# jizongFox/MI-based-Regularized-Semi-supervised-Segmentation

Measured on AMD Instinct MI355X. Metric: images/sec (UNet+IIC fwd/bwd) ACDC 256^2, higher is better.
Workload: dtype bf16; 1 GPU; udaiic train step, ACDC-shaped 1x256x256 4-class slices, LB=UB=16 per GPU, taps Conv5/Up_conv3/Up_conv2, K=20 x 5 sub-heads, paddings [1,3] (BASELINE configs[1]); mi_precision=f16f8, global_batch=32, parallelism=dp1, launch_tape=True, tape_ops=170, tape_replays_in_run=449

## Files before the change

mi-based-regularized-semi-supervised-segmentation_amd/csrc/api.hip:

```cpp
#include <stdarg.h>

#include "common.h"

namespace miseg_core {
static thread_local char g_err[512] = "";
char* last_error_buf() { return g_err; }
int fail(int code, const char* fmt, ...) {
    va_list ap;
    va_start(ap, fmt);
    vsnprintf(g_err, sizeof(g_err), fmt, ap);
    va_end(ap);
    return code;
}
}

extern "C" int miseg_version(void) { return 406; }
extern "C" const char* miseg_last_error(void) { return miseg::last_error_buf(); }

namespace miseg_core {
static hipEvent_t next_fork_event() {
    constexpr int kRing = 256, kDev = 16;
    struct Ring { hipEvent_t ev[kRing]; int made = 0, next = 0; };
    static thread_local Ring rings[kDev];
    int dev = 0;
    if (hipGetDevice(&dev) != hipSuccess || dev < 0 || dev >= kDev) return nullptr;
    Ring& r = rings[dev];
    constexpr unsigned flags = hipEventDisableTiming | hipEventDisableSystemFence;
    if (r.made < kRing) {
        if (hipEventCreateWithFlags(&r.ev[r.made], flags) != hipSuccess) return nullptr;
        ++r.made;
    }
    hipEvent_t ev = r.ev[r.next % r.made];
    r.next = (r.next + 1) % kRing;
    return ev;
}
}

extern "C" int miseg_stream_wait_stream(void* waiter, void* producer) {
    MISEG_TAPE(miseg_stream_wait_stream, waiter, producer);
    if (waiter == producer) return MISEG_OK;
    hipEvent_t ev = miseg_core::next_fork_event();
    if (!ev) return miseg_core::fail(MISEG_E_LAUNCH, "stream_wait_stream: hipEventCreateWithFlags failed");
    hipError_t e = hipEventRecord(ev, reinterpret_cast<hipStream_t>(producer));
    if (e == hipSuccess) e = hipStreamWaitEvent(reinterpret_cast<hipStream_t>(waiter), ev, 0);
    if (e != hipSuccess) return miseg_core::fail(MISEG_E_LAUNCH, "stream_wait_stream: %s", hipGetErrorString(e));
    return MISEG_OK;
}
```

mi-based-regularized-semi-supervised-segmentation_amd/csrc/conv.hip:

```cpp
#include "common.h"

namespace miseg {

constexpr int kCT = 256;
constexpr int TH = 16;
constexpr int CK = 32;

template <typename T> struct Mma;
template <> struct Mma<bf16> {
    static constexpr int CKP = 40;
    static constexpr int KP = 48;
    static constexpr int VEC = 8;
    typedef s16x8 Frag;
    static __device__ __forceinline__ Frag load(const bf16* base, int kq) { return *reinterpret_cast<const Frag*>(base + 8 * kq); }
    static __device__ __forceinline__ void mma_chunk(const Frag& a, const Frag& b, f32x4& c) {
        c = __builtin_amdgcn_mfma_f32_16x16x32_bf16(a, b, c, 0, 0, 0);
    }
};
template <> struct Mma<float> {
    static constexpr int CKP = 34;
    static constexpr int KP = 34;
    static constexpr int VEC = 4;
    struct Frag { float v[8]; };
    static __device__ __forceinline__ Frag load(const float* base, int kq) {
        Frag f;
#pragma unroll
        for (int s = 0; s < 8; ++s) f.v[s] = base[4 * s + kq];
        return f;
    }
    static __device__ __forceinline__ void mma_chunk(const Frag& a, const Frag& b, f32x4& c) {
#pragma unroll
        for (int s = 0; s < 8; ++s) c = __builtin_amdgcn_mfma_f32_16x16x4f32(a.v[s], b.v[s], c, 0, 0, 0);
    }
};

struct ConvSrc {
    const void* p0; const void* p1;
    int C0, C1, ups0, ups1;
};

template <typename T>
__device__ __forceinline__ void zero_vec(T* dst) {
#pragma unroll
    for (int i = 0; i < Mma<T>::VEC; ++i) dst[i] = from_f32<T>(0.f);
}

template <typename T, int COT, int TW, int THT, bool POOL = false, bool BNL = false, bool RED = false, int NW = 4>
__global__ __launch_bounds__(64 * NW, 1) void conv3x3_kernel(ConvSrc src, int N, int H, int W, const T* __restrict__ wpk, int Cout,
                                                        T* __restrict__ out, float* __restrict__ stats, BnFinish fin, BnLoad bl, BnRed br) {
    static_assert(!(RED && POOL), "the epilogue reduce exists for full-resolution outputs");
    typedef Mma<T> MM;
    constexpr int kCT = 64 * NW;
    static_assert(THT % NW == 0, "whole rows per wave");
    constexpr int VEC = MM::VEC, NT = COT / 16, MTR = TW / 16, RW = THT / NW, MTW = RW * MTR;
    constexpr int KP = MM::KP;
    constexpr int IW = TW + 2, IH = THT + 2;
    constexpr int NIS = (IH * IW * (CK / VEC) + kCT - 1) / kCT, NWS = (9 * COT * (CK / VEC) + kCT - 1) / kCT;
    extern __shared__ __attribute__((aligned(16))) unsigned char smem[];
    T* Is = reinterpret_cast<T*>(smem);
    T* Ws = Is + IH * IW * KP;
    const int Cin = src.C0 + src.C1;
    const int tid = threadIdx.x, lane = tid & 63, wv = tid >> 6, l15 = lane & 15, kq = lane >> 4;
    const int tilesC = (W + TW - 1) / TW, tilesR = (H + THT - 1) / THT;
    const int tc = blockIdx.x % tilesC, tr = (blockIdx.x / tilesC) % tilesR, n = blockIdx.x / (tilesC * tilesR);
    const int h0 = tr * THT, w0 = tc * TW, co0 = blockIdx.y * COT;

    f32x4 acc[MTW][NT];
#pragma unroll
    for (int m = 0; m < MTW; ++m)
#pragma unroll
        for (int t = 0; t < NT; ++t) acc[m][t] = f32x4{0.f, 0.f, 0.f, 0.f};

    uint4 pin[NIS], pwt[NWS];
    uint4 pgy[BNL ? NIS : 1];
    float cfr[BNL ? kBwdCoefRows * VEC : 1];
    unsigned okm = 0;
    static_assert(NIS <= 32 && kCT % (CK / VEC) == 0, "slot mask / per-thread channel vector");
    const uint4 zero4 = make_uint4(0u, 0u, 0u, 0u);
    auto fetch = [&](int c0) __attribute__((always_inline)) {
        if (BNL) {
            okm = 0;
            const int c = c0 + (tid % (CK / VEC)) * VEC;
#pragma unroll
// ... 370 lines not shown
                            float v = acc[m0][t][r] + acc[m1][t][r];
                            v += __shfl_xor(v, 1, 64);
                            pk[r] = from_f32<T>(v);
                        }
                        if (!mine) continue;
                        if (co + 3 < Cout) *reinterpret_cast<uint2*>(op + co) = *reinterpret_cast<const uint2*>(pk);
                        else {
#pragma unroll
                            for (int r = 0; r < 4; ++r)
                                if (co + r < Cout) op[co + r] = pk[r];
                        }
                    }
                }
            } else {
#pragma unroll
                for (int m = 0; m < MTW; ++m) {
                    const int h = h0 + wv * RW + m / MTR, w = w0 + (m % MTR) * 16 + l15;
                    const bool ok = h < H && w < W;
                    const size_t px = ((size_t)n * H + h) * W + w;
#pragma unroll
                    for (int t = 0; t < NT; ++t) {
                        const int co = co0 + t * 16 + kq * 4;
                        T* op = out + px * Cout;
                        if (fin.out1) op = co < fin.split ? out + px * fin.split : reinterpret_cast<T*>(fin.out1) + px * (Cout - fin.split) - fin.split;
                        if (ok && co + 3 < Cout) {
                            T pk[4];
#pragma unroll
                            for (int r = 0; r < 4; ++r) {
                                const float v = acc[m][t][r];
                                pk[r] = from_f32<T>(v);
                                s1[t][r] += v;
                                s2[t][r] += v * v;
                            }
                            *reinterpret_cast<uint2*>(op + co) = *reinterpret_cast<const uint2*>(pk);
                        } else if (ok) {
#pragma unroll
                            for (int r = 0; r < 4; ++r)
                                if (co + r < Cout) {
                                    const float v = acc[m][t][r];
                                    op[co + r] = from_f32<T>(v);
                                    s1[t][r] += v;
                                    s2[t][r] += v * v;
                                }
                        }
                    }
                }
            }
        }
        advance(p);
    };
    while (p.tile < t_end) {
        stage(pinA, pwtA);
        if constexpr (DEPTH == 2) {
            if (p.tile >= t_end) break;
            stage(pinB, pwtB);
        }
    }
    if (!POOL && stats) {
        __shared__ float sred[NW][2][COT];
#pragma unroll
        for (int t = 0; t < NT; ++t)
#pragma unroll
            for (int r = 0; r < 4; ++r) {
                float a = s1[t][r], b = s2[t][r];
#pragma unroll
                for (int off = 1; off < 16; off <<= 1) {
                    a += __shfl_xor(a, off, 64);
                    b += __shfl_xor(b, off, 64);
                }
                if (l15 == 0) { sred[wv][0][t * 16 + kq * 4 + r] = a; sred[wv][1][t * 16 + kq * 4 + r] = b; }
            }
        __syncthreads();
        if (tid < COT && co0 + tid < Cout) {
            float a = sred[0][0][tid] + sred[1][0][tid] + sred[2][0][tid] + sred[3][0][tid];
            float b = sred[0][1][tid] + sred[1][1][tid] + sred[2][1][tid] + sred[3][1][tid];
#pragma unroll
            for (int q = 4; q < NW; ++q) { a += sred[q][0][tid]; b += sred[q][1][tid]; }
            if (fin.acc) {
                bn_acc_add(fin.acc + co0 + tid, fin.acc + 2 * Cout, a);
                bn_acc_add(fin.acc + Cout + co0 + tid, fin.acc + 2 * Cout, b);
            } else {
                stats[((size_t)blockIdx.x * 2 + 0) * Cout + co0 + tid] = a;
                stats[((size_t)blockIdx.x * 2 + 1) * Cout + co0 + tid] = b;
            }
        }
    }
}

typedef unsigned int u32x4v __attribute__((ext_vector_type(4)));
template <int COT, int TW, int NVEC, bool DUAL, bool POOL = false, bool BNL = false, bool RED = false, int RW = 4>
__global__ __launch_bounds__(kCT, 2) void conv3x3_stream_kernel(ConvSrc src, int N, int H, int W, const bf16* __restrict__ wpk, int Cout,
                                                               bf16* __restrict__ out, float* __restrict__ stats, int ntiles, BnFinish fin,
                                                               BnLoad bl, BnRed br) {
    typedef bf16 T;
    typedef Mma<T> MM;
    static_assert(!BNL || (!DUAL && (NVEC == 1 || NVEC == 2 || NVEC == 4)), "BN loader: one source, a thread keeps one channel vector");
    static_assert(!(RED && POOL), "the epilogue reduce exists for full-resolution outputs");
    constexpr int THS = 4 * RW;
    static_assert(RW == 2 || RW == 4, "rows per wave");
    constexpr int CKP = MM::CKP, VEC = MM::VEC, NT = COT / 16, MTR = TW / 16, MTW = RW * MTR;
    constexpr int IKP = COT == 16 ? 48 : CKP;
    constexpr int IW = TW + 2, IH = THS + 2, NPIX = IH * IW;
    constexpr int NPF = DUAL ? NVEC * ((NPIX + kCT - 1) / kCT) : (NPIX * NVEC + kCT - 1) / kCT;
    constexpr unsigned OOB = 0xFFFFFF00u;
    extern __shared__ __attribute__((aligned(16))) unsigned char smem[];
    T* Is = reinterpret_cast<T*>(smem);
    T* Ws = Is + IH * IW * IKP;
    float* Cf = reinterpret_cast<float*>(Ws + 9 * COT * CKP);
    float* Rf = Cf + (BNL ? kBwdCoefRows * CK : 0);
    const int Cin = src.C0 + src.C1;
    const int tid = threadIdx.x, lane = tid & 63, wv = tid >> 6, l15 = lane & 15, kq = lane >> 4;
    const int tilesC = (W + TW - 1) / TW, tilesR = (H + THS - 1) / THS;
    const int co0 = blockIdx.y * COT;
    const int G = gridDim.x;
    const int lb = (G % 8 == 0) ? (int)(blockIdx.x % 8) * (G / 8) + (int)(blockIdx.x / 8) : (int)blockIdx.x;
    if (BNL)
        for (int idx = tid; idx < kBwdCoefRows * CK; idx += kCT) {
            const int r = idx / CK, c = idx % CK;
            Cf[idx] = c < Cin ? bl.coef[(size_t)r * Cin + c] : 0.f;
        }
    if (RED)
        for (int idx = tid; idx < 3 * COT; idx += kCT) {
            const int r = idx / COT, c = co0 + idx % COT;
            Rf[idx] = c < Cout ? br.saved[(size_t)(r == 0 ? 0 : r + 1) * Cout + c] : 0.f;
        }

    for (int idx = tid; idx < NPIX * (CK / VEC); idx += kCT) {
        const int v = idx % (CK / VEC), px = idx / (CK / VEC);
        if (v >= NVEC) zero_vec<T>(Is + px * IKP + v * VEC);
    }
    for (int idx = tid; idx < 9 * COT * (CK / VEC); idx += kCT) {
        const int v = idx % (CK / VEC), co = (idx / (CK / VEC)) % COT, tap = idx / ((CK / VEC) * COT);
        const int c = v * VEC;
        T* dst = Ws + (tap * COT + co) * CKP + v * VEC;
        if (co0 + co >= Cout || c >= Cin) { zero_vec<T>(dst); continue; }
        *reinterpret_cast<uint4*>(dst) = *reinterpret_cast<const uint4*>(wpk + ((size_t)tap * Cout + co0 + co) * Cin + c);
    }

    const int hs0 = H >> src.ups0, ws0 = W >> src.ups0, hs1 = H >> src.ups1, ws1 = W >> src.ups1;
    unsigned rel[NPF], yx[NPF];
#pragma unroll
    for (int j = 0; j < NPF; ++j) {
        int v, px;
        if (DUAL) { v = j % NVEC; px = tid + kCT * (j / NVEC); }
        else { const int idx = tid + kCT * j; v = idx % NVEC; px = idx / NVEC; }
        const int ix = px % IW, iy = px / IW, c = v * VEC;
        const bool used = px < NPIX;
        const bool from1 = c >= src.C0;
        const int ups = from1 ? src.ups1 : src.ups0, wsz = from1 ? ws1 : ws0, Cs = from1 ? src.C1 : src.C0, cs = from1 ? c - src.C0 : c;
        const int ry = ((iy - 1) >> ups) + 1, rx = ((ix - 1) >> ups) + 1;
        rel[j] = (unsigned)(((ry * wsz + rx) * Cs + cs) * 2);
        yx[j] = (used ? (unsigned)(iy | (ix << 8)) : 0xFFFFu) | ((unsigned)(used ? px * IKP + v * VEC : 0) << 16);
        static_assert(NPIX * IKP < 65536, "ldso must fit 16 bits");
    }

    if (BNL || RED) __syncthreads();
    u32x4v pf[NPF];
    u32x4v pg[BNL ? NPF : 1];
    auto fetch = [&](int tile) __attribute__((always_inline)) {
        const int tc = tile % tilesC, tr = (tile / tilesC) % tilesR, n = tile / (tilesC * tilesR);
        const int h0 = tr * THS, w0 = tc * TW;
        const int ylo = h0 == 0 ? 1 : 0, yhi = min(IH, H - h0 + 1), xlo = w0 == 0 ? 1 : 0, xhi = min(IW, W - w0 + 1);
        const long long b0 = ((((long long)n * hs0 + (h0 >> src.ups0) - 1) * ws0 + (w0 >> src.ups0) - 1) * src.C0) * 2;
        const __amdgpu_buffer_rsrc_t r0 = __builtin_amdgcn_make_buffer_rsrc((void*)((const char*)src.p0 + b0), 0, 0x7FFFFFFF, 0x00020000);
        __amdgpu_buffer_rsrc_t r1 = r0;
        if (DUAL) {
// ... 955 lines not shown
        for (int m = 0; m < ppb; ++m) t += swr[(m * G + gg) * 37 + tap * 4 + r];
        partials[(size_t)blockIdx.x * Cout * 9 + o] = t;
    }
}
__global__ __launch_bounds__(256) void stem_wgrad_sum_kernel(const float* __restrict__ partials, int nparts, int len, float* __restrict__ gw) {
    reduce_partials_block(partials, nparts, (size_t)len, len, gw, [](int e) { return (size_t)e; });
}
constexpr int kStemBlocksMax = 4096;
static const int kStemBlocks = [] { const char* e = getenv("MISEG_STEM_BLOCKS"); return e ? std::min(kStemBlocksMax, std::max(1, atoi(e))) : 1024; }();

static inline int tile_w(int64_t W) { return W >= 32 ? 32 : 16; }

}

using namespace miseg;

extern "C" int miseg_pack_conv3x3_weights(void* stream, int dt, const float* w, int64_t Cout, int64_t Cin, int kind, int64_t ci_begin,
                                          int64_t ci_count, void* packed) {
    MISEG_TAPE(miseg_pack_conv3x3_weights, stream, dt, w, Cout, Cin, kind, ci_begin, ci_count, packed);
    MISEG_F16_DISPATCH_ON(dt, miseg_pack_conv3x3_weights, stream, MISEG_BF16, w, Cout, Cin, kind, ci_begin, ci_count, packed);
    MISEG_REQUIRE(w && packed && Cout > 0 && Cin > 0, "pack_conv3x3_weights: bad args");
    MISEG_REQUIRE(kind >= 0 && (kind & 0xff) <= 1 && (kind >> 8) <= Cin && (!(kind >> 8) || !(kind & 0xff)), "pack_conv3x3_weights: bad kind");
    if (!(kind & 0xff)) { ci_begin = 0; ci_count = Cin; }
    MISEG_REQUIRE(ci_begin >= 0 && ci_count > 0 && ci_begin + ci_count <= Cin, "pack_conv3x3_weights: bad channel slice");
    const int total = (int)(9 * ((kind & 0xff) ? ci_count * Cout : Cout * Cin));
    const int nb = std::min((total + 255) / 256, 1024);
    if (dt == MISEG_F32)
        hipLaunchKernelGGL(pack_w_kernel<float>, dim3(nb), dim3(256), 0, as_stream(stream), w, (int)Cout, (int)Cin, kind, (int)ci_begin, (int)ci_count, (float*)packed);
    else if (dt == MISEG_BF16)
        hipLaunchKernelGGL(pack_w_kernel<bf16>, dim3(nb), dim3(256), 0, as_stream(stream), w, (int)Cout, (int)Cin, kind, (int)ci_begin, (int)ci_count, (bf16*)packed);
    else return fail(MISEG_E_INVALID, "pack_conv3x3_weights: bad dtype");
    MISEG_LAUNCH_CHECK("pack_w_kernel");
    return MISEG_OK;
}

extern "C" int miseg_pack_conv3x3_weights_multi(void* stream, int dt, const void* jobs_dev, int64_t njobs, int64_t total_blocks) {
    MISEG_TAPE(miseg_pack_conv3x3_weights_multi, stream, dt, jobs_dev, njobs, total_blocks);
    MISEG_F16_DISPATCH_ON(dt, miseg_pack_conv3x3_weights_multi, stream, MISEG_BF16, jobs_dev, njobs, total_blocks);
    MISEG_REQUIRE(jobs_dev && njobs > 0 && total_blocks > 0, "pack_conv3x3_weights_multi: bad args");
    static_assert(sizeof(PackJob) == 40, "PackJob layout must match miseg_pack_job");
    if (dt == MISEG_F32)
        hipLaunchKernelGGL(pack_w_multi_kernel<float>, dim3((unsigned)total_blocks), dim3(256), 0, as_stream(stream), (const PackJob*)jobs_dev, (int)njobs);
    else if (dt == MISEG_BF16)
        hipLaunchKernelGGL(pack_w_multi_kernel<bf16>, dim3((unsigned)total_blocks), dim3(256), 0, as_stream(stream), (const PackJob*)jobs_dev, (int)njobs);
    else return fail(MISEG_E_INVALID, "pack_conv3x3_weights_multi: bad dtype");
    MISEG_LAUNCH_CHECK("pack_w_multi_kernel");
    return MISEG_OK;
}

namespace miseg {
__global__ __launch_bounds__(256) void slice_cin_kernel(const float* __restrict__ src, int Cout, int Cin_pad, int Cin, float* __restrict__ dst) {
    const int total = Cout * Cin * 9;
    for (int e = blockIdx.x * 256 + threadIdx.x; e < total; e += gridDim.x * 256) {
        const int t = e % 9, ci = (e / 9) % Cin, co = e / (9 * Cin);
        dst[e] = src[((size_t)co * Cin_pad + ci) * 9 + t];
    }
}
}
extern "C" int miseg_conv3x3_wgrad_slice(void* stream, const float* gw_padded, int64_t Cout, int64_t Cin_pad, int64_t Cin, float* gw) {
    MISEG_TAPE(miseg_conv3x3_wgrad_slice, stream, gw_padded, Cout, Cin_pad, Cin, gw);
    MISEG_REQUIRE(gw_padded && gw && Cout > 0 && Cin > 0 && Cin <= Cin_pad, "conv3x3_wgrad_slice: bad args");
    const int total = (int)(Cout * Cin * 9);
    hipLaunchKernelGGL(slice_cin_kernel, dim3(std::min((total + 255) / 256, 256)), dim3(256), 0, as_stream(stream), gw_padded, (int)Cout, (int)Cin_pad,
                       (int)Cin, gw);
    MISEG_LAUNCH_CHECK("slice_cin_kernel");
    return MISEG_OK;
}

static bool conv_streams(int dt, int64_t Cin, int64_t N, int64_t H, int64_t W) {
    return dt == MISEG_BF16 && Cin <= CK && tile_w(W) == 32 && N * cdiv(H, TH) * cdiv(W, 32) >= 512;
}
static int64_t stream_blocks(int64_t N, int64_t H, int64_t W) {
    static const int64_t cap = [] { const char* e = getenv("MISEG_STREAM_BLOCKS"); return e ? atoll(e) : 512LL; }();
    return std::min<int64_t>(N * cdiv(H, TH) * cdiv(W, 32), cap);
}

struct PtGrid { int blocks, per; };
static inline PtGrid pt_grid(int ntiles, int slices, int th) {
    static const int per_cu = [] { const char* e = getenv("MISEG_PT_BLOCKS_PER_CU"); return e ? std::max(1, atoi(e)) : 2; }();
    const int target = std::max(1, (256 * (th == 8 ? per_cu : 1)) / std::max(1, slices));
    const int per = std::max(1, (ntiles + target - 1) / target);
    return PtGrid{(ntiles + per - 1) / per, per};
}
static inline bool tiled_persistent() {
    static const bool on = [] { const char* e = getenv("MISEG_CONV_PERSISTENT"); return !e || atoi(e) != 0; }();
    return on;
}

static int generic_tile_h(int dt, int64_t H, int64_t W) {
    if (dt != MISEG_BF16) return 16;
    return H * W >= 64 * 64 ? 8 : 16;
}

extern "C" int64_t miseg_conv3x3_stats_parts(int dt, int64_t Cin, int64_t N, int64_t H, int64_t W) {
    MISEG_F16_DISPATCH_ON(dt, miseg_conv3x3_stats_parts, MISEG_BF16, Cin, N, H, W);
    if (conv_streams(dt, Cin, N, H, W)) return stream_blocks(N, H, W);
    const int tw = tile_w(W);
    return N * cdiv(H, generic_tile_h(dt, H, W)) * cdiv(W, tw);
}

extern "C" int64_t miseg_conv3x3_fwd_parts(int dt, int64_t Cin, int64_t N, int64_t H, int64_t W, int64_t Cout) {
    MISEG_F16_DISPATCH_ON(dt, miseg_conv3x3_fwd_parts, MISEG_BF16, Cin, N, H, W, Cout);
    const int64_t ntiles = miseg_conv3x3_stats_parts(dt, Cin, N, H, W);
    if (conv_streams(dt, Cin, N, H, W) || dt != MISEG_BF16 || !tiled_persistent()) return ntiles;
    const int th = generic_tile_h(dt, H, W);
    if (th != 8) return ntiles;
    const int64_t cot = Cout <= 16 ? 16 : 32;
    return pt_grid((int)ntiles, (int)cdiv(Cout, cot), th).blocks;
}

static bool sumpool_supported(int dt, int64_t Cin, int64_t N, int64_t H, int64_t W, int64_t Cout) {
    if (H % 2 || W % 2) return false;
    return conv_streams(dt, Cin, N, H, W) || (dt == MISEG_BF16 && Cout > 32);
}

template <typename TT, int COT, int TWW, int THH, bool POOL>
static void launch_tiled(dim3 grid, hipStream_t st, const ConvSrc& s, int N, int H, int W, const void* wpk, int Cout, void* out, float* stats,
                         const BnFinish& fin, const BnLoad& bl, const BnRed& br) {
    const size_t lb = ((size_t)(THH + 2) * (TWW + 2) + 9 * COT) * Mma<TT>::KP * sizeof(TT);
    if constexpr (sizeof(TT) == 2) {
        if (THH == 8 && !bl.gy && !br.raw && !fin.counter && tiled_persistent()) {
            const int ntiles = (int)grid.x;
            const PtGrid g = pt_grid(ntiles, (int)grid.y, THH);
            constexpr int NWW = (THH == 16) ? 8 : 4;
            static const int depth = [] { const char* e = getenv("MISEG_CONV_DEPTH"); return e ? atoi(e) : 1; }();
            if (depth == 2 && !POOL) {
                hipFuncSetAttribute((const void*)conv3x3_pt_kernel<TT, COT, TWW, THH, POOL, NWW, 2>, hipFuncAttributeMaxDynamicSharedMemorySize, (int)lb);
                hipLaunchKernelGGL((conv3x3_pt_kernel<TT, COT, TWW, THH, POOL, NWW, 2>), dim3((unsigned)g.blocks, grid.y), dim3(64 * NWW), lb, st, s, N, H, W,
                                   (const TT*)wpk, Cout, (TT*)out, stats, fin, ntiles, g.per);
            } else {
                hipFuncSetAttribute((const void*)conv3x3_pt_kernel<TT, COT, TWW, THH, POOL, NWW, 1>, hipFuncAttributeMaxDynamicSharedMemorySize, (int)lb);
                hipLaunchKernelGGL((conv3x3_pt_kernel<TT, COT, TWW, THH, POOL, NWW, 1>), dim3((unsigned)g.blocks, grid.y), dim3(64 * NWW), lb, st, s, N, H, W,
                                   (const TT*)wpk, Cout, (TT*)out, stats, fin, ntiles, g.per);
            }
            return;
        }
    }
#define GO(BNL, RED, NWW)                                                                                                            \
    {                                                                                                                               \
        hipFuncSetAttribute((const void*)conv3x3_kernel<TT, COT, TWW, THH, POOL, BNL, RED, NWW>, hipFuncAttributeMaxDynamicSharedMemorySize, (int)lb); \
        hipLaunchKernelGGL((conv3x3_kernel<TT, COT, TWW, THH, POOL, BNL, RED, NWW>), grid, dim3(64 * NWW), lb, st, s, N, H, W, (const TT*)wpk, \
                           Cout, (TT*)out, stats, fin, bl, br);                                                                     \
    }
    if constexpr (THH == 16 && sizeof(TT) == 2) {
        if (!bl.gy && !br.raw) { GO(false, false, 8) return; }
    }
    if constexpr (POOL) { if (bl.gy) GO(true, false, 4) else GO(false, false, 4) }
    else { if (bl.gy && br.raw) GO(true, true, 4) else if (bl.gy) GO(true, false, 4) else if (br.raw) GO(false, true, 4) else GO(false, false, 4) }
#undef GO
}
template <int COT, int NV, bool POOL> constexpr int fused_rw() { return (NV == 2 && (COT == 16 || POOL)) ? 4 : 2; }
template <int COT, int NV, bool DU, bool POOL>
static int launch_stream(unsigned blocks, hipStream_t st, const ConvSrc& s, int N, int H, int W, const void* wpk, int Cout, void* out, float* stats,
                         const BnFinish& fin, const BnLoad& bl, const BnRed& br) {
    const dim3 grid(blocks, (unsigned)cdiv(Cout, COT));
#define GO(BNL, RED, RWW)                                                                                                            \
    {                                                                                                                               \
        const size_t lb = ((size_t)(4 * RWW + 2) * (32 + 2) * (COT == 16 ? 48 : Mma<bf16>::CKP) + 9 * COT * Mma<bf16>::CKP) * sizeof(bf16) + \
                          (BNL ? kBwdCoefRows * CK * 4 : 0) + (RED ? 3 * COT * 4 : 0);                                               \
        const int ntiles = (int)(N * cdiv(H, 4 * RWW) * cdiv(W, 32));                                                                \
        hipFuncSetAttribute((const void*)conv3x3_stream_kernel<COT, 32, NV, DU, POOL, BNL, RED, RWW>, hipFuncAttributeMaxDynamicSharedMemorySize, (int)lb); \
        hipLaunchKernelGGL((conv3x3_stream_kernel<COT, 32, NV, DU, POOL, BNL, RED, RWW>), grid, dim3(kCT), lb, st, s, N, H, W,          \
                           (const bf16*)wpk, Cout, (bf16*)out, stats, ntiles, fin, bl, br);                                          \
    }
    constexpr bool kFusable = !DU && (NV == 2 || NV == 4);
    if constexpr (kFusable) {
        constexpr int FRW = fused_rw<COT, NV, POOL>();
        if constexpr (POOL) { if (bl.gy) GO(true, false, FRW) else GO(false, false, 4) }
        else { if (bl.gy && br.raw) GO(true, true, FRW) else if (bl.gy) GO(true, false, FRW) else if (br.raw) GO(false, true, FRW) else GO(false, false, 4) }
    } else {
        if (bl.gy || br.raw) return fail(MISEG_E_INVALID, "conv3x3: BatchNorm loader / reduce not built for this streaming shape");
        GO(false, false, 4)
    }
#undef GO
    return MISEG_OK;
}

static int conv3x3_fwd_impl(void* stream, int dt, const void* in0, int64_t C0, int ups0, const void* in1, int64_t C1, int ups1,
                            int64_t N, int64_t H, int64_t W, const void* packed_w, int64_t Cout, void* out, float* stats, BnFinish fin,
                            bool pool_out = false, BnLoad bl = BnLoad{nullptr, nullptr}, BnRed br = BnRed{nullptr, nullptr, nullptr}) {
    MISEG_REQUIRE(in0 && packed_w && out, "conv3x3_fwd: null pointer");
    MISEG_REQUIRE(N > 0 && H > 0 && W > 0 && Cout > 0 && C0 > 0 && C1 >= 0, "conv3x3_fwd: bad shape");
    MISEG_REQUIRE(C1 == 0 || in1, "conv3x3_fwd: second source missing");
    MISEG_REQUIRE((ups0 == 0 || ups0 == 1) && (ups1 == 0 || ups1 == 1), "conv3x3_fwd: ups must be 0/1");
    MISEG_REQUIRE((!ups0 || (H % 2 == 0 && W % 2 == 0)) && (!ups1 || (H % 2 == 0 && W % 2 == 0)), "conv3x3_fwd: upsampled size must be even");
    const int vec = dt == MISEG_BF16 ? 8 : 4;
    MISEG_REQUIRE(C0 % vec == 0 && C1 % vec == 0, "conv3x3_fwd: channel counts must be multiples of %d (use conv_small for the stem)", vec);
    ConvSrc s{in0, in1, (int)C0, (int)C1, ups0, ups1};
    const int tw = tile_w(W);
    const int th = conv_streams(dt, C0 + C1, N, H, W) ? TH : generic_tile_h(dt, H, W);
    const unsigned gx = (unsigned)(N * cdiv(H, th) * cdiv(W, tw));
    hipStream_t st = as_stream(stream);
    MISEG_REQUIRE(!bl.gy || (bl.coef && C1 == 0 && ups0 == 0), "conv3x3: the BatchNorm loader reads one full-resolution source");
    MISEG_REQUIRE(!br.raw || (br.saved && br.parts && !pool_out && !stats && Cout % 4 == 0), "conv3x3: epilogue reduce needs a full-resolution "
                  "output with a multiple of 4 channels and no forward statistics");
#define LAUNCH_TH(TT, COT, TWW, THH)                                                                                       \
    launch_tiled<TT, COT, TWW, THH, false>(dim3(gx, (unsigned)cdiv(Cout, COT)), st, s, (int)N, (int)H, (int)W, packed_w, (int)Cout, out, stats, fin, bl, br);
#define LAUNCH(TT, COT, TWW) { if (th == 8) LAUNCH_TH(TT, COT, TWW, 8) else LAUNCH_TH(TT, COT, TWW, 16) }
    MISEG_REQUIRE(!pool_out || (sumpool_supported(dt, C0 + C1, N, H, W, Cout) && C1 == 0 && !stats),
                  "conv3x3_fwd_sumpool: shape not supported (ask miseg_conv3x3_fwd_sumpool_supported)");
    if (conv_streams(dt, C0 + C1, N, H, W)) {
        int rc = MISEG_OK;
#define SLAUNCH(COT, NV, DU)                                                                                               \
    {                                                                                                                     \
        const unsigned g = (unsigned)stream_blocks(N, H, W);                                                               \
        if (pool_out && !DU) rc = launch_stream<COT, NV, false, true>(g, st, s, (int)N, (int)H, (int)W, packed_w, (int)Cout, out, stats, fin, bl, br); \
        else rc = launch_stream<COT, NV, DU, false>(g, st, s, (int)N, (int)H, (int)W, packed_w, (int)Cout, out, stats, fin, bl, br); \
    }
#define SLAUNCH_NV(COT)                                                                                                    \
    {                                                                                                                     \
        if (C1 > 0) { switch ((C0 + C1) / 8) { case 2: SLAUNCH(COT, 2, true) break; case 3: SLAUNCH(COT, 3, true) break; default: SLAUNCH(COT, 4, true) break; } } \
        else { switch (C0 / 8) { case 1: SLAUNCH(COT, 1, false) break; case 2: SLAUNCH(COT, 2, false) break; case 3: SLAUNCH(COT, 3, false) break; default: SLAUNCH(COT, 4, false) break; } } \
    }
        if (Cout <= 16) SLAUNCH_NV(16)
        else SLAUNCH_NV(32)
#undef SLAUNCH_NV
#undef SLAUNCH
        if (rc != MISEG_OK) return rc;
    } else if (dt == MISEG_BF16 && pool_out) {
#define LAUNCH_P(TWW, THH)                                                                                                 \
    launch_tiled<bf16, 64, TWW, THH, true>(dim3(gx, (unsigned)cdiv(Cout, 64)), st, s, (int)N, (int)H, (int)W, packed_w, (int)Cout, out, stats, fin, bl, br);
        if (tw == 32) { if (th == 8) LAUNCH_P(32, 8) else LAUNCH_P(32, 16) }
        else { if (th == 8) LAUNCH_P(16, 8) else LAUNCH_P(16, 16) }
#undef LAUNCH_P
    } else if (dt == MISEG_BF16) {
// ... 293 lines not shown
```

Before: 4947 images/s.

## Add double-buffered tiled 3x3 conv kernel overlapping global loads with MFMA

Adds a new tiled conv3x3 kernel that keeps two shared-memory buffers, one per input-channel chunk. Global loads for chunk k+2 are issued into registers and committed to the spare buffer tap by tap while MFMAs run on the current chunk, so there is one barrier per chunk. It is enabled by default (through an env toggle) for 16-row, 16-bit tiled convs that have no BN loader, no reduce and no counter. The cost is roughly double the LDS footprint at one block per CU and extra register pressure from the staged loads. A standalone per-layer benchmark script is also added.

```diff
diff --git a/mi-based-regularized-semi-supervised-segmentation_amd/csrc/api.hip b/mi-based-regularized-semi-supervised-segmentation_amd/csrc/api.hip
--- a/mi-based-regularized-semi-supervised-segmentation_amd/csrc/api.hip
+++ b/mi-based-regularized-semi-supervised-segmentation_amd/csrc/api.hip
@@ -14,7 +14,7 @@
 }
 }
 
-extern "C" int miseg_version(void) { return 406; }
+extern "C" int miseg_version(void) { return 407; }
 extern "C" const char* miseg_last_error(void) { return miseg::last_error_buf(); }
 
 namespace miseg_core {
diff --git a/mi-based-regularized-semi-supervised-segmentation_amd/csrc/conv.hip b/mi-based-regularized-semi-supervised-segmentation_amd/csrc/conv.hip
--- a/mi-based-regularized-semi-supervised-segmentation_amd/csrc/conv.hip
+++ b/mi-based-regularized-semi-supervised-segmentation_amd/csrc/conv.hip
@@ -1,4 +1,5 @@
 #include "common.h"
+#include <type_traits>
 
 namespace miseg {
 
@@ -535,6 +536,238 @@
             } else {
                 stats[((size_t)blockIdx.x * 2 + 0) * Cout + co0 + tid] = a;
                 stats[((size_t)blockIdx.x * 2 + 1) * Cout + co0 + tid] = b;
+            }
+        }
+    }
+}
+
+template <typename T, int COT, int TW, int THT, bool POOL, int NW>
+__global__ __launch_bounds__(64 * NW, 1) void conv3x3_db_kernel(ConvSrc src, int N, int H, int W, const T* __restrict__ wpk, int Cout,
+                                                           T* __restrict__ out, float* __restrict__ stats, BnFinish fin) {
+    static_assert(sizeof(T) == 2, "double-buffered tiled form: 16-bit storage types");
+    typedef Mma<T> MM;
+    constexpr int kCT = 64 * NW;
+    static_assert(THT % NW == 0, "whole rows per wave");
+    constexpr int VEC = MM::VEC, CV4 = CK / VEC, NT = COT / 16, MTR = TW / 16, RW = THT / NW, MTW = RW * MTR;
+    constexpr int KS = CK;
+    constexpr int IW = TW + 2, IH = THT + 2;
+    constexpr int NIS = (IH * IW * CV4 + kCT - 1) / kCT, NWS = (9 * COT * CV4 + kCT - 1) / kCT, NSL = NIS + NWS;
+    constexpr int RPS = kCT / CV4;
+    static_assert(RPS % 8 == 0 && RPS % COT == 0 && NIS <= 16 && NWS <= 16, "slot j of a thread: same swizzle term, same output channel as slot 0");
+    constexpr int IMG = (IH * IW + 9 * COT) * KS;
+    static_assert((IH * IW) % 4 == 0 && NSL <= 18, "the weight block starts on a 256-byte bank row; two slots per tap");
+    extern __shared__ __attribute__((aligned(16))) unsigned char smem[];
+    T* S = reinterpret_cast<T*>(smem);
+    const int Cin = src.C0 + src.C1;
+    const int tid = threadIdx.x, lane = tid & 63, wv = tid >> 6, l15 = lane & 15, kq = lane >> 4;
+    const int tilesC = (W + TW - 1) / TW, tilesR = (H + THT - 1) / THT;
+    const int tc = blockIdx.x % tilesC, tr = (blockIdx.x / tilesC) % tilesR, n = blockIdx.x / (tilesC * tilesR);
+    const int h0 = tr * THT, w0 = tc * TW, co0 = blockIdx.y * COT;
+    const int nck = (Cin + CK - 1) / CK;
+
+    const int cv = (tid % CV4) * VEC, row0 = tid / CV4;
+    const int sofs = row0 * KS + (cv ^ ((((row0 >> 2) & 1) << 1) * VEC));
+    int i_rel0[NIS], i_rel1[NIS];
+    unsigned okm = 0, wkm = 0;
+    {
+        const int ws0 = W >> src.ups0, ws1 = W >> src.ups1;
+#pragma unroll
+        for (int j = 0; j < NIS; ++j) {
+            const int px = row0 + RPS * j, h = h0 - 1 + px / IW, w = w0 - 1 + px % IW;
+            if (px < IH * IW && h >= 0 && h < H && w >= 0 && w < W) okm |= 1u << j;
+            i_rel0[j] = ((h >> src.ups0) * ws0 + (w >> src.ups0)) * src.C0 + cv;
+            i_rel1[j] = ((h >> src.ups1) * ws1 + (w >> src.ups1)) * src.C1 + cv - src.C0;
+        }
+#pragma unroll
+        for (int j = 0; j < NWS; ++j)
+            if (row0 + RPS * j < 9 * COT && co0 + row0 % COT < Cout) wkm |= 1u << j;
+    }
+    const T* s0n = reinterpret_cast<const T*>(src.p0) + (size_t)n * (H >> src.ups0) * (W >> src.ups0) * src.C0;
+    const T* s1n = reinterpret_cast<const T*>(src.p1) + (size_t)n * (H >> src.ups1) * (W >> src.ups1) * src.C1;
+    const T* wrow = wpk + ((size_t)(row0 / COT) * Cout + co0 + row0 % COT) * Cin + cv;
+    const size_t wstep = (size_t)(RPS / COT) * Cout * Cin;
+
+    uint4 pin[NIS], pwt[NWS];
+    auto slot_ok = [&](int s, int c0) __attribute__((always_inline)) {
+        return (s < NIS ? (okm >> s) & 1u : (wkm >> (s - NIS)) & 1u) && c0 + cv < Cin;
+    };
+    auto fetch_slot = [&](int s, int c0) __attribute__((always_inline)) {
+        const bool ok = slot_ok(s, c0);
+        if (s < NIS) {
+            const bool first = c0 + cv < src.C0;
+            const T* a = ok ? (first ? s0n + i_rel0[s] : s1n + i_rel1[s]) + c0 : s0n;
+            pin[s] = *reinterpret_cast<const uint4*>(a);
+        } else {
+            const int j = s - NIS;
+            const T* a = ok ? wrow + j * wstep + c0 : wpk;
+            pwt[j] = *reinterpret_cast<const uint4*>(a);
+        }
+    };
+    auto keep = [](bool ok, const uint4& q) __attribute__((always_inline)) {
+        return make_uint4(ok ? q.x : 0u, ok ? q.y : 0u, ok ? q.z : 0u, ok ? q.w : 0u);
+    };
+    auto commit_slot = [&](int s, int c0, T* img) __attribute__((always_inline)) {
+        const bool ok = slot_ok(s, c0);
+        if (s < NIS) {
+            if (row0 + RPS * s < IH * IW) *reinterpret_cast<uint4*>(img + sofs + s * RPS * KS) = keep(ok, pin[s]);
+        } else {
+            const int j = s - NIS;
+            if (row0 + RPS * j < 9 * COT) *reinterpret_cast<uint4*>(img + IH * IW * KS + sofs + j * RPS * KS) = keep(ok, pwt[j]);
+        }
+    };
+    int ibase[8];
+    {
+        const int R0 = wv * RW * IW + l15;
+#pragma unroll
+        for (int c7 = 0; c7 < 8; ++c7) {
+            const int r = R0 + c7;
+            ibase[c7] = r * KS + ((kq ^ (((r >> 2) & 1) << 1)) * VEC);
+        }
+    }
+    const int wbase = IH * IW * KS + l15 * KS + ((kq ^ (((l15 >> 2) & 1) << 1)) * VEC);
+
+    f32x4 acc[MTW][NT];
+#pragma unroll
+    for (int m = 0; m < MTW; ++m)
+#pragma unroll
+        for (int t = 0; t < NT; ++t) acc[m][t] = f32x4{0.f, 0.f, 0.f, 0.f};
+
+#pragma unroll
+    for (int s = 0; s < NSL; ++s) fetch_slot(s, 0);
+#pragma unroll
+    for (int s = 0; s < NSL; ++s) commit_slot(s, 0, S);
+    if (nck > 1) {
+#pragma unroll
+        for (int s = 0; s < NSL; ++s) fetch_slot(s, CK);
+    }
+    __syncthreads();
+    auto body = [&](int k, auto wr_c, auto ld_c) __attribute__((always_inline)) {
+        constexpr bool WR = decltype(wr_c)::value, LD = decltype(ld_c)::value;
+        const T* cur = S + (k & 1) * IMG;
+        T* nxt = S + ((k + 1) & 1) * IMG;
+#pragma unroll
+        for (int tap = 0; tap < 9; ++tap) {
+            if constexpr (WR) {
+#pragma unroll
+                for (int s = 0; s < NSL; ++s)
+                    if (8 - (NSL - 1 - s) / 2 == tap) {
+                        commit_slot(s, (k + 1) * CK, nxt);
+                        if constexpr (LD) fetch_slot(s, (k + 2) * CK);
+                    }
+            }
+            const int ky = tap / 3, kx = tap % 3;
+            typename MM::Frag bf[NT];
+#pragma unroll
+            for (int t = 0; t < NT; ++t) bf[t] = *reinterpret_cast<const typename MM::Frag*>(cur + wbase + (tap * COT + t * 16) * KS);
+#pragma unroll
+            for (int m = 0; m < MTW; ++m) {
+                const int c = (m / MTR + ky) * IW + (m % MTR) * 16 + kx;
+                typename MM::Frag af = *reinterpret_cast<const typename MM::Frag*>(cur + ibase[c & 7] + (c & ~7) * KS);
+#pragma unroll
+                for (int t = 0; t < NT; ++t) MM::mma_chunk(bf[t], af, acc[m][t]);
+            }
+        }
+        __syncthreads();
+    };
+    {
+        int k = 0;
+        for (; k + 2 < nck; ++k) body(k, std::true_type{}, std::true_type{});
+        if (k + 1 < nck) body(k++, std::true_type{}, std::false_type{});
+        body(k, std::false_type{}, std::false_type{});
+    }
+    if (POOL) {
+        static_assert(!POOL || RW % 2 == 0, "pooled epilogue: a wave owns whole row pairs");
+        const int Hp = H >> 1, Wp = W >> 1;
+#pragma unroll
+        for (int mp = 0; mp < MTW / 2; ++mp) {
+            const int m0 = (2 * (mp / MTR)) * MTR + mp % MTR, m1 = m0 + MTR;
+            const int hp = ((h0 + wv * RW) >> 1) + mp / MTR, wp = ((w0 + (mp % MTR) * 16) >> 1) + (l15 >> 1);
+            const bool mine = !(l15 & 1) && hp < Hp && wp < Wp;
+            T* op = out + (((size_t)n * Hp + hp) * Wp + wp) * Cout;
+#pragma unroll
+            for (int t = 0; t < NT; ++t) {
+                const int co = co0 + t * 16 + kq * 4;
+                T pk[4];
+#pragma unroll
+                for (int r = 0; r < 4; ++r) {
+                    float v = acc[m0][t][r] + acc[m1][t][r];
+                    v += __shfl_xor(v, 1, 64);
+                    pk[r] = from_f32<T>(v);
+                }
+                if (!mine) continue;
+                if (co + 3 < Cout) *reinterpret_cast<uint2*>(op + co) = *reinterpret_cast<const uint2*>(pk);
+                else {
+#pragma unroll
+                    for (int r = 0; r < 4; ++r)
+                        if (co + r < Cout) op[co + r] = pk[r];
+                }
+            }
+        }
+        return;
+    }
+    float s1[NT][4], s2[NT][4];
+#pragma unroll
+    for (int t = 0; t < NT; ++t)
+#pragma unroll
+        for (int r = 0; r < 4; ++r) s1[t][r] = s2[t][r] = 0.f;
+#pragma unroll
+    for (int m = 0; m < MTW; ++m) {
+        const int h = h0 + wv * RW + m / MTR, w = w0 + (m % MTR) * 16 + l15;
+        const bool ok = h < H && w < W;
+        const size_t px = ((size_t)n * H + h) * W + w;
+#pragma unroll
+        for (int t = 0; t < NT; ++t) {
+            const int co = co0 + t * 16 + kq * 4;
+            T* op = out + px * Cout;
+            if (fin.out1) op = co < fin.split ? out + px * fin.split : reinterpret_cast<T*>(fin.out1) + px * (Cout - fin.split) - fin.split;
+            if (ok && co + 3 < Cout) {
+                T pk[4];
+#pragma unroll
+                for (int r = 0; r < 4; ++r) {
+                    const float v = acc[m][t][r];
+                    pk[r] = from_f32<T>(v);
+                    s1[t][r] += v;
+                    s2[t][r] += v * v;
+                }
+                *reinterpret_cast<uint2*>(op + co) = *reinterpret_cast<const uint2*>(pk);
+            } else if (ok) {
+#pragma unroll
+                for (int r = 0; r < 4; ++r)
+                    if (co + r < Cout) {
+                        const float v = acc[m][t][r];
+                        op[co + r] = from_f32<T>(v);
+                        s1[t][r] += v;
+                        s2[t][r] += v * v;
+                    }
+            }
+        }
+    }
+    if (stats) {
+        __shared__ float sred[NW][2][COT];
+#pragma unroll
+        for (int t = 0; t < NT; ++t)
+#pragma unroll
+            for (int r = 0; r < 4; ++r) {
+                float a = s1[t][r], b = s2[t][r];
+#pragma unroll
+                for (int off = 1; off < 16; off <<= 1) {
+                    a += __shfl_xor(a, off, 64);
+                    b += __shfl_xor(b, off, 64);
+                }
+                if (l15 == 0) { sred[wv][0][t * 16 + kq * 4 + r] = a; sred[wv][1][t * 16 + kq * 4 + r] = b; }
+            }
+        __syncthreads();
+        if (tid < COT && co0 + tid < Cout) {
+            float a = sred[0][0][tid] + sred[1][0][tid] + sred[2][0][tid] + sred[3][0][tid];
+            float b = sred[0][1][tid] + sred[1][1][tid] + sred[2][1][tid] + sred[3][1][tid];
+#pragma unroll
+            for (int q = 4; q < NW; ++q) { a += sred[q][0][tid]; b += sred[q][1][tid]; }
+            if (fin.acc) {
+                bn_acc_add(fin.acc + co0 + tid, fin.acc + 2 * Cout, a);
+                bn_acc_add(fin.acc + Cout + co0 + tid, fin.acc + 2 * Cout, b);
+            } else {
+                store_part(&stats[((size_t)blockIdx.x * 2 + 0) * Cout + co0 + tid], a);
+                store_part(&stats[((size_t)blockIdx.x * 2 + 1) * Cout + co0 + tid], b);
             }
         }
     }
@@ -1656,6 +1889,10 @@
     const int per = std::max(1, (ntiles + target - 1) / target);
     return PtGrid{(ntiles + per - 1) / per, per};
 }
+static inline bool tiled_pipeline() {
+    const char* e = getenv("MISEG_CONV_PIPELINE");
+    return !e || atoi(e) != 0;
+}
 static inline bool tiled_persistent() {
     static const bool on = [] { const char* e = getenv("MISEG_CONV_PERSISTENT"); return !e || atoi(e) != 0; }();
     return on;
@@ -1715,6 +1952,15 @@
         hipFuncSetAttribute((const void*)conv3x3_kernel<TT, COT, TWW, THH, POOL, BNL, RED, NWW>, hipFuncAttributeMaxDynamicSharedMemorySize, (int)lb); \
         hipLaunchKernelGGL((conv3x3_kernel<TT, COT, TWW, THH, POOL, BNL, RED, NWW>), grid, dim3(64 * NWW), lb, st, s, N, H, W, (const TT*)wpk, \
                            Cout, (TT*)out, stats, fin, bl, br);                                                                     \
+    }
+    if constexpr (THH == 16 && sizeof(TT) == 2) {
+        if (!bl.gy && !br.raw && !fin.counter && tiled_pipeline()) {
+            const size_t lb2 = 2 * ((size_t)(THH + 2) * (TWW + 2) + 9 * COT) * CK * sizeof(TT);
+            hipFuncSetAttribute((const void*)conv3x3_db_kernel<TT, COT, TWW, THH, POOL, 8>, hipFuncAttributeMaxDynamicSharedMemorySize, (int)lb2);
+            hipLaunchKernelGGL((conv3x3_db_kernel<TT, COT, TWW, THH, POOL, 8>), grid, dim3(64 * 8), lb2, st, s, N, H, W, (const TT*)wpk, Cout,
+                               (TT*)out, stats, fin);
+            return;
+        }
     }
     if constexpr (THH == 16 && sizeof(TT) == 2) {
         if (!bl.gy && !br.raw) { GO(false, false, 8) return; }
diff --git a/profiles/conv_tiled_bench.py b/profiles/conv_tiled_bench.py
--- /dev/null
+++ b/profiles/conv_tiled_bench.py
@@ -0,0 +1,89 @@
+import argparse
+import json
+import os
+import sys
+
+import torch
+
+ROOT = os.path.dirname(os.path.dirname(os.path.abspath(__file__)))
+sys.path.insert(0, os.path.join(ROOT, "mi-based-regularized-semi-supervised-segmentation_amd"))
+from miseg_amd import _cabi
+
+SHAPES = [
+    ("Conv3.1 fwd", 64, 32, 0, 0, 0, 64, "acc"), ("Conv3.2 fwd", 64, 64, 0, 0, 0, 64, "acc"),
+    ("Conv4.1 fwd", 32, 64, 0, 0, 0, 128, "acc"), ("Conv4.2 fwd", 32, 128, 0, 0, 0, 128, "acc"),
+    ("Conv5.1 fwd", 16, 128, 0, 0, 0, 256, "acc"), ("Conv5.2 fwd", 16, 256, 0, 0, 0, 256, "acc"),
+    ("Up5 fwd", 32, 256, 1, 0, 0, 128, "acc"), ("Up_conv5.1 fwd", 32, 128, 0, 128, 0, 128, "acc"), ("Up_conv5.2 fwd", 32, 128, 0, 0, 0, 128, "acc"),
+    ("Up4 fwd", 64, 128, 1, 0, 0, 64, "acc"), ("Up_conv4.1 fwd", 64, 64, 0, 64, 0, 64, "acc"), ("Up_conv4.2 fwd", 64, 64, 0, 0, 0, 64, "acc"),
+    ("Up_conv4.2 dgrad", 64, 64, 0, 0, 0, 64, "plain"), ("Up_conv4.1 dgrad", 64, 64, 0, 0, 0, 128, "split"), ("Up4 dgrad", 64, 64, 0, 0, 0, 128, "pool"),
+    ("Up_conv5.2 dgrad", 32, 128, 0, 0, 0, 128, "plain"), ("Up_conv5.1 dgrad", 32, 128, 0, 0, 0, 256, "split"), ("Up5 dgrad", 32, 128, 0, 0, 0, 256, "pool"),
+    ("Conv5.2 dgrad", 16, 256, 0, 0, 0, 256, "plain"), ("Conv5.1 dgrad", 16, 256, 0, 0, 0, 128, "plain"),
+    ("Conv4.2 dgrad", 32, 128, 0, 0, 0, 128, "plain"), ("Conv4.1 dgrad", 32, 128, 0, 0, 0, 64, "plain"),
+    ("Conv3.2 dgrad", 64, 64, 0, 0, 0, 64, "plain"), ("Conv3.1 dgrad", 64, 64, 0, 0, 0, 32, "plain"),
+]
+
+
+def main():
+    ap = argparse.ArgumentParser()
+    ap.add_argument("--dtype", default="bf16", choices=["bf16", "f16"])
+    ap.add_argument("--n", type=int, default=48)
+    ap.add_argument("--launches", type=int, default=20)
+    ap.add_argument("--warmup", type=int, default=5)
+    ap.add_argument("--out", default=None)
+    a = ap.parse_args()
+    dtype, dt = (torch.bfloat16, _cabi.BF16) if a.dtype == "bf16" else (torch.float16, _cabi.F16)
+    dev = "cuda"
+    st = torch.cuda.current_stream().cuda_stream
+    g = torch.Generator(device=dev).manual_seed(0)
+    big = torch.randn(6144, 6144, device=dev, dtype=torch.bfloat16, generator=g)
+    rows = []
+    print(f"# lib version {_cabi.lib().miseg_version()} MISEG_CONV_PIPELINE={os.environ.get('MISEG_CONV_PIPELINE')} "
+          f"{a.dtype} N={a.n}: {a.launches} launches after {a.warmup} warm-ups")
+    for name, hw, c0, u0, c1, u1, cout, form in SHAPES:
+        n, cin = a.n, c0 + c1
+        x0 = torch.randn(n, hw >> u0, hw >> u0, c0, device=dev, generator=g).to(dtype)
+        x1 = torch.randn(n, hw >> u1, hw >> u1, c1, device=dev, generator=g).to(dtype) if c1 else None
+        wpk = (torch.randn(9 * cout * cin, device=dev, generator=g) * (2.0 / (9 * cin)) ** 0.5).to(dtype)
+        p1 = x1.data_ptr() if c1 else None
+        if form == "acc":
+            out = torch.empty(n, hw, hw, cout, device=dev, dtype=dtype)
+            acc = torch.zeros(2 * cout + 1, device=dev, dtype=torch.int64)
+            fn = lambda: _cabi.call("miseg_conv3x3_fwd_acc", st, dt, x0.data_ptr(), c0, u0, p1, c1, u1, n, hw, hw, wpk.data_ptr(), cout,
+                                    out.data_ptr(), acc.data_ptr())
+        elif form == "plain":
+            out = torch.empty(n, hw, hw, cout, device=dev, dtype=dtype)
+            fn = lambda: _cabi.call("miseg_conv3x3_fwd", st, dt, x0.data_ptr(), c0, u0, p1, c1, u1, n, hw, hw, wpk.data_ptr(), cout, out.data_ptr(), None)
+        elif form == "pool":
+            out = torch.empty(n, hw // 2, hw // 2, cout, device=dev, dtype=dtype)
+            fn = lambda: _cabi.call("miseg_conv3x3_fwd_sumpool", st, dt, x0.data_ptr(), c0, n, hw, hw, wpk.data_ptr(), cout, out.data_ptr())
+        else:
+            out = torch.empty(n, hw, hw, cout // 2, device=dev, dtype=dtype)
+            out1 = torch.empty(n, hw, hw, cout // 2, device=dev, dtype=dtype)
+            fn = lambda: _cabi.call("miseg_conv3x3_dgrad_dual", st, dt, x0.data_ptr(), c0, n, hw, hw, wpk.data_ptr(), cout // 2, out.data_ptr(),
+                                    cout // 2, out1.data_ptr())
+        for _ in range(a.warmup):
+            fn()
+        torch.cuda.synchronize()
+        e0, e1 = torch.cuda.Event(enable_timing=True), torch.cuda.Event(enable_timing=True)
+        torch.mm(big, big)
+        e0.record()
+        for _ in range(a.launches):
+            fn()
+        e1.record()
+        torch.cuda.synchronize()
+        us = e0.elapsed_time(e1) * 1e3 / a.launches
+        gf = 18.0 * cin * cout * n * hw * hw / 1e9
+        rows.append({"layer": name, "hw": hw, "cin": cin, "cout": cout, "form": form, "gflop": round(gf, 2), "us": round(us, 2),
+                     "tflops": round(gf / us * 1e3, 1)})
+        print(f"{name:18s} {hw:3d}^2 {cin:3d}->{cout:3d} {form:5s} {gf:6.2f} GF {us:7.2f} us {gf / us * 1e3:7.1f} TFLOP/s")
+    tot = sum(r["us"] for r in rows)
+    print(f"sum {tot:.1f} us over {len(rows)} launches")
+    if a.out:
+        os.makedirs(os.path.dirname(os.path.abspath(a.out)), exist_ok=True)
+        with open(a.out, "w") as f:
+            json.dump({"lib_version": int(_cabi.lib().miseg_version()), "dtype": a.dtype, "n": a.n, "pipeline": os.environ.get("MISEG_CONV_PIPELINE"),
+                       "rows": rows, "sum_us": round(tot, 1)}, f, indent=1)
+
+
+if __name__ == "__main__":
+    main()
```

Result: no change. 4918 images/s, median of 2 (-0.6%).
